# nv-tlabs/DefTet

Measured on AMD Instinct MI355X. Metric: M tet-point tests/s (fwd+bwd) at res=70, 100k queries, higher is better.
Workload: dtype f32

## Files before the change

### deftet_amd/csrc/point_in_tet.hip

```cpp
#pragma clang fp contract(off)

#include <stdlib.h>

#include <algorithm>
#include <type_traits>
#include <vector>

#include "common.hpp"

namespace deftet {
namespace pit {

constexpr float kBig = 1048576.0f;
constexpr float kTau = 1.0f / 128.0f;
constexpr float kMargin = 1.0f / 64.0f;
constexpr float kWMin = 9.3132257e-10f;
constexpr int kMiss = 0x7F7F7F7F;
constexpr int kMaxG = 112;
constexpr int kMaxBins = 15 * 1024;
constexpr int kHitOverflow = -2;

constexpr int kHitPad = 64;
__host__ __device__ inline int hit_pad(int B) { return (B + kHitPad - 1) / kHitPad * kHitPad; }
__host__ __device__ inline size_t hit_cnt_off(int B, int T) { return (size_t)B * T * 2; }
// ... 662 lines not shown
    PHASE_MARK(12);
    SPAN_MARK(1);
    if (keep) return;
    __syncthreads();
    for (int i = tid; i < n; i += kSortThreads) {
        const float4 q = src[source_of(i)];
        dst[atomicAdd(&cnt[(cell_of(q.y, oy, iy, G) - cyLo) * GxP + cell_of(q.x, ox, ix, Gx)], 1)] = q;
    }
}

__device__ __forceinline__ void irregular_queries_tail(const Planes &P, int t, int b, int Q, const float *__restrict__ pts,
                                                       const int *__restrict__ counters, const int *__restrict__ irregQ, int *result)
{
    const int n = counters[b * 4 + 1];
    for (int k = 0; k < n; ++k) {
        const int q = irregQ[(size_t)b * Q + k];
        const float *p = pts + ((size_t)b * Q + q) * 3;
        if (accept(P, p[0], p[1], p[2])) atomicMin(&result[(size_t)b * Q + q], t);
    }
}

#ifndef PIT_WAVES
#define PIT_WAVES 5
#endif


struct TetBox {
    float lo[3], hi[3], w;
};
__device__ __forceinline__ bool classify(const float *v, const Planes &P, TetBox &bx)
{
#pragma unroll
    for (int k = 0; k < 3; ++k) {
        bx.lo[k] = fminf(fminf(v[k], v[3 + k]), fminf(v[6 + k], v[9 + k]));
        bx.hi[k] = fmaxf(fmaxf(v[k], v[3 + k]), fmaxf(v[6 + k], v[9 + k]));
    }
    bx.w = fmaxf(fmaxf(bx.hi[0] - bx.lo[0], bx.hi[1] - bx.lo[1]), bx.hi[2] - bx.lo[2]);
    const float big = fmaxf(fmaxf(fmaxf(fabsf(bx.lo[0]), fabsf(bx.hi[0])), fmaxf(fabsf(bx.lo[1]), fabsf(bx.hi[1]))),
                            fmaxf(fabsf(bx.lo[2]), fabsf(bx.hi[2])));
    const float thr = kTau * ((bx.w * bx.w) * bx.w);
    const bool cond = fabsf(P.dv[0]) >= thr && fabsf(P.dv[1]) >= thr && fabsf(P.dv[2]) >= thr && fabsf(P.dv[3]) >= thr;
    return big <= kBig && (P.sv == 0u || P.sv == 15u) && bx.w >= kWMin && cond;
}

struct CellBox {
    int cx0, cx1, cy0, cy1, cz0, cz1;
};

__device__ __forceinline__ float4 ld_f4_hint(const float4 *p, bool nt)
{
    if (!nt) return *p;
    typedef float f4v __attribute__((ext_vector_type(4)));
    const f4v x = __builtin_nontemporal_load(reinterpret_cast<const f4v *>(p));
    return make_float4(x[0], x[1], x[2], x[3]);
}
struct DenseTets {
    typedef const float *__restrict__ Arg;
    typedef const float *Ref;
    typedef const float *__restrict__ RefArg;
    const float *tet;
    __host__ __device__ __forceinline__ DenseTets(const float *p) : tet(p) {}
    __device__ __forceinline__ Ref at(int b, int T, int t) const { return tet + ((size_t)b * T + t) * 12; }
    __device__ __forceinline__ Ref at_flat(long long i, int ) const { return tet + i * 12; }
    template <bool NT = false>
    __device__ __forceinline__ static void get3(Ref r, float4 &a, float4 &bq, float4 &c)
    {
        const float4 *src = reinterpret_cast<const float4 *>(r);
        a = ld_f4_hint(src, NT); bq = ld_f4_hint(src + 1, NT); c = ld_f4_hint(src + 2, NT);
    }
    template <bool NT = false>
    __device__ __forceinline__ static void get4(Ref r, float (&v)[12])
    {
        float4 a, bq, c;
        get3<NT>(r, a, bq, c);
        v[0] = a.x; v[1] = a.y; v[2] = a.z; v[3] = a.w;
        v[4] = bq.x; v[5] = bq.y; v[6] = bq.z; v[7] = bq.w;
        v[8] = c.x; v[9] = c.y; v[10] = c.z; v[11] = c.w;
    }
    __device__ __forceinline__ static void get(Ref r, float (&v)[12])
    {
#pragma unroll
        for (int k = 0; k < 12; ++k) v[k] = r[k];
    }
};
struct IndexedTets {
    const float *pos;
    const int *idx;
    long long idxStride;
    int V;
    typedef IndexedTets Arg;
    struct Ref {
        const float *p;
        const int *ix;
        unsigned V;
    };
    typedef Ref RefArg;
    __device__ __forceinline__ Ref at(int b, int T, int t) const
    {
        (void)T;
        return Ref{pos + (size_t)b * (size_t)V * 3, idx + (size_t)b * idxStride + (size_t)t * 4, (unsigned)V};
    }
    __device__ __forceinline__ Ref at_flat(long long i, int T) const { return at((int)(i / T), T, (int)(i % T)); }
    template <bool NT = false>
    __device__ __forceinline__ static void get4(const Ref &r, float (&v)[12])
    {
        const int4 c = *reinterpret_cast<const int4 *>(r.ix);
        const int ci[4] = {c.x, c.y, c.z, c.w};
#pragma unroll
        for (int k = 0; k < 4; ++k) {
            const unsigned u = (unsigned)ci[k];
            if (u < r.V) {
                const float *p = r.p + (size_t)u * 3;
                v[3 * k] = p[0]; v[3 * k + 1] = p[1]; v[3 * k + 2] = p[2];
            } else {
                v[3 * k] = v[3 * k + 1] = v[3 * k + 2] = __int_as_float(0x7FC00000);
            }
        }
    }
    template <bool NT = false>
    __device__ __forceinline__ static void get3(const Ref &r, float4 &a, float4 &bq, float4 &c)
    {
        float v[12];
        get4(r, v);
        a = make_float4(v[0], v[1], v[2], v[3]); bq = make_float4(v[4], v[5], v[6], v[7]); c = make_float4(v[8], v[9], v[10], v[11]);
    }
    __device__ __forceinline__ static void get(const Ref &r, float (&v)[12]) { get4(r, v); }
};
__global__ __launch_bounds__(256) void k_idx_check(const int4 *__restrict__ idx, long long n, unsigned V, int *bad)
{
    const long long i = (long long)blockIdx.x * blockDim.x + threadIdx.x;
    if (i >= n) return;
    const int4 c = idx[i];
    if ((unsigned)c.x >= V || (unsigned)c.y >= V || (unsigned)c.z >= V || (unsigned)c.w >= V) *bad = 1;
}

template <class TS_, bool F>
struct TetCfg {
    typedef TS_ TS;
    static constexpr bool flag = F;
};

template <class TS>
__global__ __launch_bounds__(256, PIT_WAVES) void k_tet_scan(typename TS::Arg tet, int T, int Q,
                                                  const float *__restrict__ gparam, int G, int Gx, const int *__restrict__ table,
                                                  long long cellStride, const float4 *__restrict__ sortedQ, int *result, int *counters,
                                                  int *irregT, int2 *hits, const float *__restrict__ pts,
                                                  const int *__restrict__ irregQ, int *ucount, int hpad, int4 *spill)
{
    if (ucount && blockIdx.x == 0 && __builtin_amdgcn_readfirstlane(threadIdx.x) == 0) {
        ucount[blockIdx.y] = 0;
        ucount[hpad + blockIdx.y] = 0;
        ucount[2 * hpad + blockIdx.y] = 0;
    }
    const int b = blockIdx.y;
    const int nblk = gridDim.x;
    const int per = (nblk + 7) >> 3;
    const int vb = (blockIdx.x & 7) * per + (blockIdx.x >> 3);
    const int t = vb * blockDim.x + threadIdx.x;
    if (vb >= nblk || t >= T) return;
    const TS ts(tet);
    float v[12];
    if constexpr (std::is_same<TS, DenseTets>::value) {
        const float4 *src = reinterpret_cast<const float4 *>(tet + ((size_t)b * T + t) * 12);
        float4 a = src[0], bq = src[1], c = src[2];
        v[0] = a.x; v[1] = a.y; v[2] = a.z; v[3] = a.w;
        v[4] = bq.x; v[5] = bq.y; v[6] = bq.z; v[7] = bq.w;
        v[8] = c.x; v[9] = c.y; v[10] = c.z; v[11] = c.w;
    } else {
        TS::get4(ts.at(b, T, t), v);
    }
    Planes P;
    make_planes(v, P);
    TetBox bx;
    const bool regular = classify(v, P, bx);
    int hq[kRecSlots + kSpillSlots] = {-1, -1, -1, -1, -1, -1};
    int hcnt = 0;
    if (!regular) {
        int k = atomicAdd(&counters[b * 4 + 0], 1);
        irregT[(size_t)b * T + k] = t;
        if (hits) hits[(size_t)b * T + t] = make_int2(-1, kHitOverflow);
        irregular_queries_tail(P, t, b, Q, pts, counters, irregQ, result);
        return;
    }
    const Grid g = load_grid(gparam + b * kGridWords);
    const float m = bx.w * kMargin;
    float elo[3], ehi[3];
#pragma unroll
    for (int k = 0; k < 3; ++k) {
        elo[k] = bx.lo[k] - m;
        ehi[k] = bx.hi[k] + m;
    }
    if (ehi[0] < g.lo[0] || elo[0] > g.hi[0] || ehi[1] < g.lo[1] || elo[1] > g.hi[1] || ehi[2] < g.lo[2] || elo[2] > g.hi[2]) {
        if (hits) hits[(size_t)b * T + t] = make_int2(-1, -1);
        irregular_queries_tail(P, t, b, Q, pts, counters, irregQ, result);
        return;
    }
    const int cx0 = cell_of(elo[0], g.o[0], g.inv[0], Gx), cx1 = cell_of(ehi[0], g.o[0], g.inv[0], Gx);
    const int cy0 = cell_of(elo[1], g.o[1], g.inv[1], G), cy1 = cell_of(ehi[1], g.o[1], g.inv[1], G);
    const int cz0 = cell_of(elo[2], g.o[2], g.inv[2], G), cz1 = cell_of(ehi[2], g.o[2], g.inv[2], G);
    if (wide_tet(cx0, cx1, cy0, cy1, cz0, cz1, g)) {
        int k = atomicAdd(&counters[b * 4 + 0], 1);
        irregT[(size_t)b * T + k] = t;
        if (hits) hits[(size_t)b * T + t] = make_int2(-1, kHitOverflow);
        irregular_queries_tail(P, t, b, Q, pts, counters, irregQ, result);
        return;
    }
    const int Gp = table_pitch(G);
    const int *tb = table + (size_t)b * cellStride;
    const float4 *sq = sortedQ + (size_t)b * Q;
    int *res = result + (size_t)b * Q;
    for (int cz = cz0; cz <= cz1; ++cz)
        for (int cy = cy0; cy <= cy1; ++cy) {
            const int s = tb[table_off(cz, cx0, cy, Gx, Gp)], e = tb[table_off(cz, cx1 + 1, cy, Gx, Gp)];
            for (int j = s; j < e; ++j) {
                const float4 q = sq[j];
                if (q.x >= elo[0] && q.x <= ehi[0] && q.y >= elo[1] && q.y <= ehi[1] && q.z >= elo[2] && q.z <= ehi[2] &&
                    accept(P, q.x, q.y, q.z)) {
                    const int qi = __float_as_int(q.w);
                    atomicMin(&res[qi], t);
#pragma unroll
                    for (int k = 0; k < kRecSlots + kSpillSlots; ++k)
                        if (hcnt == k) hq[k] = qi;
                    ++hcnt;
                }
            }
        }
    if (hits) put_hit_record(hits, spill, (size_t)b * T + t, hq, hcnt, counters, gridDim.y, b, t);
    irregular_queries_tail(P, t, b, Q, pts, counters, irregQ, result);
}

struct Filter {
    float N[4][3];
    float C[4];
    float twoEmax;
};

typedef unsigned long long lanemask_t;
__device__ __forceinline__ int sel(lanemask_t m, int if_set, int if_clear)
{
    int d;
    asm("v_cndmask_b32_e64 %0, %1, %2, %3" : "=v"(d) : "v"(if_clear), "v"(if_set), "s"(m));
    return d;
}
__device__ __forceinline__ unsigned sel(lanemask_t m, unsigned if_set, unsigned if_clear)
{
    return (unsigned)sel(m, (int)if_set, (int)if_clear);
}
__device__ __forceinline__ lanemask_t mask_of(bool c) { return __builtin_amdgcn_ballot_w64(c); }


template <typename T>
__device__ __forceinline__ T ld_off(const void *base, unsigned byte_off)
{
    return *reinterpret_cast<const T *>(static_cast<const char *>(base) + byte_off);
}
struct __attribute__((packed, aligned(4))) int4u { int x, y, z, w; };
__device__ __forceinline__ int4u ld_off_u4(const void *base, unsigned byte_off)
{
    return *reinterpret_cast<const int4u *>(static_cast<const char *>(base) + byte_off);
}

__device__ __forceinline__ void atomic_smin_off(int *base, unsigned byte_off, int v)
{
    asm volatile("s_nop 4\n\tglobal_atomic_smin %0, %1, %2" ::"v"(byte_off), "v"(v), "s"(base) : "memory");
}
template <typename T>
__device__ __forceinline__ T *uniform_ptr(T *p)
{
    const unsigned long long v = reinterpret_cast<unsigned long long>(p);
    const unsigned lo = __builtin_amdgcn_readfirstlane((unsigned)v), hi = __builtin_amdgcn_readfirstlane((unsigned)(v >> 32));
    return reinterpret_cast<T *>(((unsigned long long)hi << 32) | lo);
}
typedef int i32x4 __attribute__((ext_vector_type(4)));
typedef int i32x2s __attribute__((ext_vector_type(2)));
typedef float f32x4 __attribute__((ext_vector_type(4)));
__device__ __forceinline__ void stream_store(float4 *p, const float4 v)
{
    const f32x4 x = {v.x, v.y, v.z, v.w};
    __builtin_nontemporal_store(x, reinterpret_cast<f32x4 *>(p));
}
__device__ __forceinline__ void stream_store(float *p, float v) { __builtin_nontemporal_store(v, p); }
#ifndef PIT_SCAN_TET_NT
#define PIT_SCAN_TET_NT 0
#endif
#ifndef PIT_BWD_TET_NT
#define PIT_BWD_TET_NT 0
#endif
#ifndef PIT_BWD_REV
#define PIT_BWD_REV 0
#endif
#ifndef PIT_REC_NT
#define PIT_REC_NT 1
#endif
__device__ __forceinline__ void store_rec(int2 *p, const int2 v)
{
    if (PIT_REC_NT) {
        const i32x2s x = {v.x, v.y};
        __builtin_nontemporal_store(x, reinterpret_cast<i32x2s *>(p));
    } else {
        *p = v;
    }
}
__device__ __forceinline__ int2 stream_load(const int2 *p)
{
    const i32x2s x = __builtin_nontemporal_load(reinterpret_cast<const i32x2s *>(p));
    return make_int2(x.x, x.y);
}
__device__ __forceinline__ void store_b128_off(void *base, unsigned byte_off, int x, int y, int z, int w)
{
    const i32x4 v = {x, y, z, w};
    asm volatile("s_nop 4\n\tglobal_store_dwordx4 %0, %1, %2\n\ts_nop 2" ::"v"(byte_off), "v"(v), "s"(base) : "memory");
}

typedef int i32x2 __attribute__((ext_vector_type(2)));
__device__ __forceinline__ void store_b64_off(void *base, unsigned byte_off, int x, int y)
{
    const i32x2 v = {x, y};
    asm volatile("s_nop 4\n\tglobal_store_dwordx2 %0, %1, %2\n\ts_nop 2" ::"v"(byte_off), "v"(v), "s"(base) : "memory");
}

template <class TS>
__device__ __noinline__ void exact_rescan(typename TS::RefArg tv, int t, const int *__restrict__ tb, const float4 *__restrict__ sq,
                                          int *res, int G, int Gx, int cx0, int cx1, int cy0, int cy1, int cz0, int cz1,
                                          float m, int *counters, int nB, int b, int2 *hits, int4 *spill, size_t idx)
{
    float vv[12];
    TS::get(tv, vv);
    Planes P;
    make_planes(vv, P);
    float elo[3], ehi[3];
#pragma unroll
    for (int k = 0; k < 3; ++k) {
        elo[k] = fminf(fminf(vv[k], vv[3 + k]), fminf(vv[6 + k], vv[9 + k])) - m;
        ehi[k] = fmaxf(fmaxf(vv[k], vv[3 + k]), fmaxf(vv[6 + k], vv[9 + k])) + m;
    }
    const int Gp = table_pitch(G);
    int hq[kRecSlots + kSpillSlots] = {-1, -1, -1, -1, -1, -1};
    int hcnt = 0;
    for (int cz = cz0; cz <= cz1; ++cz)
// ... 1287 lines not shown
        if (threadIdx.x == 0) {
            const float tot = (wsum[0] + wsum[1]) + (wsum[2] + wsum[3]);
            if (tot != 0.f) unsafeAtomicAdd(&missSum[b], tot);
        }
    }
}

template <class TS>
__global__ __launch_bounds__(256) void k_bary_bwd_gather(typename TS::Arg tet, const float *__restrict__ pts,
                                                         const float *__restrict__ grad_w, const int *__restrict__ head,
                                                         const int *__restrict__ next, int T, int Q, float *grad_tet,
                                                         float *grad_pts, int accumulate, const float *__restrict__ gocc,
                                                         const float *__restrict__ missSum, float *grad_pred)
{
    const int b = blockIdx.y;
    const int t = blockIdx.x * blockDim.x + threadIdx.x;
    if (t >= T) return;
    float acc[12];
#pragma unroll
    for (int k = 0; k < 12; ++k) acc[k] = 0.f;
    int q = head[(size_t)b * T + t];
    float gp = (grad_pred && t == 0) ? missSum[b] : 0.f;
    if (q >= 0) {
        float4 t0, t1, t2;
        TS::get3(TS(tet).at(b, T, t), t0, t1, t2);
        const float A[3] = {t0.x, t0.y, t0.z}, Bv[3] = {t0.w, t1.x, t1.y}, Cv[3] = {t1.z, t1.w, t2.x}, D[3] = {t2.y, t2.z, t2.w};
        float vab[3], vac[3], vad[3], vbc[3], vbd[3];
#pragma unroll
        for (int k = 0; k < 3; ++k) {
            vab[k] = Bv[k] - A[k]; vac[k] = Cv[k] - A[k]; vad[k] = D[k] - A[k];
            vbc[k] = Cv[k] - Bv[k]; vbd[k] = D[k] - Bv[k];
        }
        float na[3], nb[3], nc[3], nd[3];
        cross3(vbd, vbc, na);
        cross3(vac, vad, nb);
        cross3(vad, vab, nc);
        cross3(vab, vac, nd);
        const float v6 = 1.0f / (vab[0] * nb[0] + vab[1] * nb[1] + vab[2] * nb[2]);
        while (q >= 0) {
            const size_t i = (size_t)b * Q + q;
            const float *pp = pts + i * 3;
            const float4 g = reinterpret_cast<const float4 *>(grad_w)[i];
            const int qn = next[i];
            float vap[3], vbp[3];
#pragma unroll
            for (int k = 0; k < 3; ++k) { vap[k] = pp[k] - A[k]; vbp[k] = pp[k] - Bv[k]; }
            float w[4];
            w[0] = (vbp[0] * na[0] + vbp[1] * na[1] + vbp[2] * na[2]) * v6;
            w[1] = (vap[0] * nb[0] + vap[1] * nb[1] + vap[2] * nb[2]) * v6;
            w[2] = (vap[0] * nc[0] + vap[1] * nc[1] + vap[2] * nc[2]) * v6;
            w[3] = (vap[0] * nd[0] + vap[1] * nd[1] + vap[2] * nd[2]) * v6;
            float G3[3];
#pragma unroll
            for (int k = 0; k < 3; ++k) G3[k] = (g.x * na[k] + g.y * nb[k] + g.z * nc[k] + g.w * nd[k]) * v6;
#pragma unroll
            for (int vtx = 0; vtx < 4; ++vtx)
#pragma unroll
                for (int k = 0; k < 3; ++k) acc[vtx * 3 + k] += -w[vtx] * G3[k];
            if (grad_pts) { grad_pts[i * 3] = G3[0]; grad_pts[i * 3 + 1] = G3[1]; grad_pts[i * 3 + 2] = G3[2]; }
            if (grad_pred) gp += gocc[i];
            q = qn;
        }
    }
    if (grad_pred) grad_pred[(size_t)b * T + t] = accumulate ? grad_pred[(size_t)b * T + t] + gp : gp;
    float4 *dst = reinterpret_cast<float4 *>(grad_tet + ((size_t)b * T + t) * 12);
    float4 o0 = make_float4(acc[0], acc[1], acc[2], acc[3]), o1 = make_float4(acc[4], acc[5], acc[6], acc[7]),
           o2 = make_float4(acc[8], acc[9], acc[10], acc[11]);
    if (accumulate) {
        float4 p0 = dst[0], p1 = dst[1], p2 = dst[2];
        o0.x += p0.x; o0.y += p0.y; o0.z += p0.z; o0.w += p0.w;
        o1.x += p1.x; o1.y += p1.y; o1.z += p1.z; o1.w += p1.w;
        o2.x += p2.x; o2.y += p2.y; o2.z += p2.z; o2.w += p2.w;
    }
    dst[0] = o0; dst[1] = o1; dst[2] = o2;
}

constexpr int kMissParts = 64;

struct TetGrad {
    float A[3], Bv[3];
    float na[3], nb[3], nc[3], nd[3];
    float v6;
};
template <class TS>
__device__ __forceinline__ void tet_grad_setup(typename TS::Ref r, TetGrad &g)
{
    float4 t0, t1, t2;
    TS::template get3<PIT_BWD_TET_NT != 0>(r, t0, t1, t2);
    const float C[3] = {t1.z, t1.w, t2.x}, D[3] = {t2.y, t2.z, t2.w};
    g.A[0] = t0.x; g.A[1] = t0.y; g.A[2] = t0.z; g.Bv[0] = t0.w; g.Bv[1] = t1.x; g.Bv[2] = t1.y;
    float vab[3], vac[3], vad[3], vbc[3], vbd[3];
#pragma unroll
    for (int k = 0; k < 3; ++k) {
        vab[k] = g.Bv[k] - g.A[k]; vac[k] = C[k] - g.A[k]; vad[k] = D[k] - g.A[k];
        vbc[k] = C[k] - g.Bv[k]; vbd[k] = D[k] - g.Bv[k];
    }
    cross3(vbd, vbc, g.na);
    cross3(vac, vad, g.nb);
    cross3(vad, vab, g.nc);
    cross3(vab, vac, g.nd);
    g.v6 = 1.0f / (vab[0] * g.nb[0] + vab[1] * g.nb[1] + vab[2] * g.nb[2]);
}
__device__ __forceinline__ void tet_grad_add(const TetGrad &g, const float *pp, const float4 gw, float *acc, float *G3)
{
    float vap[3], vbp[3];
#pragma unroll
    for (int k = 0; k < 3; ++k) { vap[k] = pp[k] - g.A[k]; vbp[k] = pp[k] - g.Bv[k]; }
    float w[4];
    w[0] = (vbp[0] * g.na[0] + vbp[1] * g.na[1] + vbp[2] * g.na[2]) * g.v6;
    w[1] = (vap[0] * g.nb[0] + vap[1] * g.nb[1] + vap[2] * g.nb[2]) * g.v6;
    w[2] = (vap[0] * g.nc[0] + vap[1] * g.nc[1] + vap[2] * g.nc[2]) * g.v6;
    w[3] = (vap[0] * g.nd[0] + vap[1] * g.nd[1] + vap[2] * g.nd[2]) * g.v6;
#pragma unroll
    for (int k = 0; k < 3; ++k) G3[k] = (gw.x * g.na[k] + gw.y * g.nb[k] + gw.z * g.nc[k] + gw.w * g.nd[k]) * g.v6;
#pragma unroll
    for (int vtx = 0; vtx < 4; ++vtx)
#pragma unroll
        for (int k = 0; k < 3; ++k) acc[vtx * 3 + k] += -w[vtx] * G3[k];
}

__device__ __forceinline__ float mem_read_f32(float *p) { return __int_as_float(atomicOr(reinterpret_cast<int *>(p), 0)); }
__device__ __forceinline__ void mem_write_f32(float *p, float v)
{
    const int old = atomicExch(reinterpret_cast<int *>(p), __float_as_int(v));
    asm volatile("" ::"v"(old));
}

constexpr int kMissStride = 80;

constexpr long long kRescanOrderedSteps = 16384;
template <class TS>
__device__ __forceinline__ bool bwd_rescan(typename TS::Arg tet, const float *__restrict__ pts, const float *__restrict__ cond,
                                        const float *__restrict__ grad_w, const float *__restrict__ gocc, float *grad_pts,
                                        bool want_pred, const int *__restrict__ ulist, int b, int T, int Q, int nU,
                                        unsigned long long need, int t, float (*park)[256])
{
    const int tid = threadIdx.x, lane = tid & 63;
    const int *__restrict__ lst = ulist + (size_t)b * Q;
    bool parked = false;
    while (need) {
        const int L = __ffsll((long long)need) - 1;
        need &= need - 1;
        const int tL = __shfl(t, L);
        const float tLf = (float)tL;
        int m = 0;
        auto next_hit = [&](int cur, bool count) {
            int best = 0x7FFFFFFF;
            for (int base = 0; base < nU; base += 64) {
                const int e = base + lane;
                const int q = e < nU ? lst[e] : -1;
                const bool mine = q > cur && cond[(size_t)b * Q + q] == tLf;
                if (mine) best = min(best, q);
                if (count) m += __popcll(__ballot(mine));
            }
#pragma unroll
            for (int off = 32; off > 0; off >>= 1) best = min(best, __shfl_xor(best, off));
            return best;
        };
        int best = next_hit(-1, true);
        if (m == 0) continue;
        const bool ordered = (long long)m * ((nU + 63) >> 6) <= kRescanOrderedSteps;
        float part[13];
#pragma unroll
        for (int k = 0; k < 13; ++k) part[k] = 0.f;
        TetGrad g;
        tet_grad_setup<TS>(TS(tet).at(b, T, tL), g);
        for (int base = 0;;) {
            int q;
            bool mine;
            if (ordered) {
                if (best == 0x7FFFFFFF) break;
                q = best;
                mine = true;
            } else {
                if (base >= nU) break;
                const int e = base + lane;
                q = e < nU ? lst[e] : -1;
                mine = q >= 0 && cond[(size_t)b * Q + q] == tLf;
                base += 64;
            }
            if (mine) {
                const size_t i = (size_t)b * Q + q;
                float G3[3];
                tet_grad_add(g, pts + i * 3, reinterpret_cast<const float4 *>(grad_w)[i], part, G3);
                if (grad_pts) { grad_pts[i * 3] = G3[0]; grad_pts[i * 3 + 1] = G3[1]; grad_pts[i * 3 + 2] = G3[2]; }
                if (want_pred) part[12] += gocc[i];
            }
            if (ordered) best = next_hit(best, false);
        }
        if (!ordered) {
#pragma unroll
            for (int k = 0; k < 13; ++k) {
                float v = part[k];
#pragma unroll
                for (int off = 32; off > 0; off >>= 1) v += __shfl_xor(v, off);
                part[k] = v;
            }
        }
        if (lane == L) {
#pragma unroll
            for (int k = 0; k < 13; ++k) park[k][tid] = part[k];
            parked = true;
        }
    }
    return parked;
}

#ifndef PIT_BWD_WAVES
#define PIT_BWD_WAVES 7
#endif
template <class C>
__global__ __launch_bounds__(256, PIT_BWD_WAVES) void k_bary_bwd_hits(typename C::TS::Arg tet, const float *__restrict__ pts,
                                                       const float *__restrict__ cond, const float *__restrict__ grad_w,
                                                       const int2 *__restrict__ hits, int T, int Q, float *grad_tet,
                                                       float *grad_pts, int accumulate, const float *__restrict__ gocc,
                                                       float *grad_pred, float *missPart, int nMissParts, int *hitWords,
                                                       const int *__restrict__ ulist, int pad, const int4 *__restrict__ spill, int pin,
                                                       unsigned long long *rowMask)
{
    __shared__ float wsum[4];
    __shared__ float s_vals[kMissStride];
    __shared__ int s_last;
    __shared__ __attribute__((aligned(16))) float s_buf[13 * 256];
    float4(*s_rows)[192] = reinterpret_cast<float4(*)[192]>(s_buf);
    float(*s_park)[256] = reinterpret_cast<float(*)[256]>(s_buf);
    typedef typename C::TS TS;
    constexpr bool SPARSE = C::flag;
    const int2 sb = shape_block(pin);
    const int b = sb.x, bx = PIT_BWD_REV ? (int)gridDim.x - 1 - sb.y : sb.y, tid = threadIdx.x, lane = tid & 63;
    const bool side = grad_pred && bx < nMissParts;
    float missPartial = 0.f;
    if (side) {
        float gm = 0.f;
        for (int q = bx * blockDim.x + tid; q < Q; q += nMissParts * blockDim.x)
            if (cond[(size_t)b * Q + q] < 0.f) gm += gocc[(size_t)b * Q + q];
#pragma unroll
        for (int off = 32; off > 0; off >>= 1) gm += __shfl_xor(gm, off);
        if (lane == 0) wsum[tid >> 6] = gm;
        __syncthreads();
        missPartial = __int_as_float(__builtin_amdgcn_readfirstlane(__float_as_int((wsum[0] + wsum[1]) + (wsum[2] + wsum[3]))));
    }
    const int t = bx * blockDim.x + tid;
    const bool live = t < T;
    int2 h = live ? stream_load(hits + (size_t)b * T + t) : make_int2(-1, -1);
    const bool spilled = h.y != kHitOverflow && h.x >= 0 && (h.x & kHitSpilled) != 0;
    if (spilled) h.x &= ~kHitSpilled;
    bool parked = false;
    const int nU = hitWords[b];
    if (nU > 0) {
        const bool anyQ = hitWords[2 * pad + b] != 0;
        const unsigned long long need = __ballot(live && (h.y == kHitOverflow || anyQ));
        if (need) parked = bwd_rescan<TS>(tet, pts, cond, grad_w, gocc, grad_pts, grad_pred != nullptr, ulist, b, T, Q, nU, need, t, s_park);
    }
    float acc[12];
#pragma unroll
    for (int k = 0; k < 12; ++k) acc[k] = 0.f;
    float gp = 0.f;
    if (h.x >= 0 && h.y != kHitOverflow) {
        TetGrad g;
        tet_grad_setup<TS>(TS(tet).at(b, T, t), g);
        unsigned hu[8] = {(unsigned)h.x, (unsigned)h.y, ~0u, ~0u, ~0u, ~0u, ~0u, ~0u};
        const float tf = (float)t;
        auto add_hit = [&](int q) {
            if (q < 0) return;
            const size_t i = (size_t)b * Q + q;
            const float c = cond[i], go = grad_pred ? gocc[i] : 0.f;
            const float pq[3] = {pts[i * 3], pts[i * 3 + 1], pts[i * 3 + 2]};
            const float4 gw = reinterpret_cast<const float4 *>(grad_w)[i];
            const bool won = c == tf;
            float G3[3], a2[12];
#pragma unroll
            for (int k = 0; k < 12; ++k) a2[k] = acc[k];
            tet_grad_add(g, pq, gw, a2, G3);
#pragma unroll
            for (int k = 0; k < 12; ++k) acc[k] = won ? a2[k] : acc[k];
            if (won && grad_pts) { grad_pts[i * 3] = G3[0]; grad_pts[i * 3 + 1] = G3[1]; grad_pts[i * 3 + 2] = G3[2]; }
            gp = won ? gp + go : gp;
        };
#define DEFTET_CSWAP(a, b) { const unsigned lo_ = min(hu[a], hu[b]), hi_ = max(hu[a], hu[b]); hu[a] = lo_; hu[b] = hi_; }
        if (!__any(spilled)) {
            DEFTET_CSWAP(0, 1)
#pragma unroll 1
            for (int k = 0; k < 2 && __any(hu[0] != ~0u); ++k) {
                add_hit((int)hu[0]);
                hu[0] = hu[1]; hu[1] = ~0u;
            }
        } else {
            if (spilled) {
                const int4 h2 = spill[(size_t)b * T + t];
                hu[2] = (unsigned)h2.x; hu[3] = (unsigned)h2.y; hu[4] = (unsigned)h2.z; hu[5] = (unsigned)h2.w;
            }
            DEFTET_CSWAP(0, 1) DEFTET_CSWAP(2, 3) DEFTET_CSWAP(4, 5) DEFTET_CSWAP(6, 7)
            DEFTET_CSWAP(0, 2) DEFTET_CSWAP(1, 3) DEFTET_CSWAP(4, 6) DEFTET_CSWAP(5, 7)
            DEFTET_CSWAP(1, 2) DEFTET_CSWAP(5, 6) DEFTET_CSWAP(0, 4) DEFTET_CSWAP(3, 7)
            DEFTET_CSWAP(1, 5) DEFTET_CSWAP(2, 6)
            DEFTET_CSWAP(1, 4) DEFTET_CSWAP(3, 6)
            DEFTET_CSWAP(2, 4) DEFTET_CSWAP(3, 5)
            DEFTET_CSWAP(3, 4)
#pragma unroll 1
            for (int k = 0; k < 6 && __any(hu[0] != ~0u); ++k) {
                add_hit((int)hu[0]);
#pragma unroll
                for (int j = 0; j < 7; ++j) hu[j] = hu[j + 1];
                hu[7] = ~0u;
            }
        }
#undef DEFTET_CSWAP
    }
    if (parked) {
#pragma unroll
        for (int k = 0; k < 12; ++k) acc[k] += s_park[k][tid];
        gp += s_park[12][tid];
    }
    if (nU > 0) __syncthreads();
    if (live) {
        const bool deferred = grad_pred && t == 0;
        if (grad_pred && !deferred) stream_store(grad_pred + (size_t)b * T + t, accumulate ? grad_pred[(size_t)b * T + t] + gp : gp);
    }
    {
        const int w = tid >> 6;
        const int t0 = t - lane;
        const bool has = live && ((h.x >= 0 && h.y != kHitOverflow) || parked);
        const unsigned long long hm = SPARSE ? __ballot(has) : 0ull;
        const int slot = SPARSE ? __popcll(hm & ((1ull << lane) - 1ull)) : lane;
        if (!SPARSE || has) {
            s_rows[w][slot * 3] = make_float4(acc[0], acc[1], acc[2], acc[3]);
            s_rows[w][slot * 3 + 1] = make_float4(acc[4], acc[5], acc[6], acc[7]);
            s_rows[w][slot * 3 + 2] = make_float4(acc[8], acc[9], acc[10], acc[11]);
        }
        if (SPARSE && lane == 0 && t0 < T) rowMask[(size_t)b * ((T + 63) >> 6) + (t0 >> 6)] = hm;
        __syncthreads();
        float4 *dst = reinterpret_cast<float4 *>(grad_tet + ((size_t)b * T + t0) * 12);
        const int nRow = (SPARSE ? __popcll(hm) : min(64, T - t0)) * 3;
#pragma unroll
        for (int k = 0; k < 3; ++k) {
            const int j = k * 64 + lane;
            if (j < nRow) {
                float4 o = s_rows[w][j];
                if (accumulate && !SPARSE) { const float4 p = dst[j]; o.x += p.x; o.y += p.y; o.z += p.z; o.w += p.w; }
                stream_store(dst + j, o);
            }
        }
    }
    if (!side) return;
    float *mp = missPart + (size_t)b * kMissStride;
    int *ticket = hitWords + pad + b;
    if (tid == 0) {
        mem_write_f32(mp + bx, missPartial);
        if (bx == 0) mem_write_f32(mp + kMissParts, gp);
        __builtin_amdgcn_s_waitcnt(0);
        s_last = atomicAdd(ticket, 1) == nMissParts - 1;
    }
    __syncthreads();
    if (!s_last) return;
    if (tid <= kMissParts) s_vals[tid] = (tid < nMissParts || tid == kMissParts) ? mem_read_f32(mp + tid) : 0.f;
    __syncthreads();
    if (tid == 0) {
        float tot = 0.f;
        for (int k = 0; k < kMissParts; ++k) tot += s_vals[k];
        tot += s_vals[kMissParts];
        float *dst = grad_pred + (size_t)b * T;
        *dst = accumulate ? *dst + tot : tot;
        atomicExch(ticket, 0);
    }
}

__global__ __launch_bounds__(256) void k_paste_fwd(const float *__restrict__ pred, float *cond, float *out, int T, int Q,
                                                   int clamp_inplace)
{
    const int b = blockIdx.y;
    const int q = blockIdx.x * blockDim.x + threadIdx.x;
    if (q >= Q) return;
    const size_t i = (size_t)b * Q + q;
    float c = cond[i];
    if (c < 0) {
        c = 0.f;
        if (clamp_inplace) cond[i] = 0.f;
    }
    out[i] = pred[(size_t)b * T + (long long)c];
}

__global__ __launch_bounds__(256) void k_paste_bwd(const float *__restrict__ cond, const float *__restrict__ gout,
                                                   float *gpred, int T, int Q)
{
    const int b = blockIdx.y;
    const int q = blockIdx.x * blockDim.x + threadIdx.x;
    const bool live = q < Q;
// ... 348 lines not shown
{
    int n = 0;
    DEFTET_HIP(hipOccupancyMaxActiveBlocksPerMultiprocessor(&n, (const void *)deftet::pit::k_tet_scan_wave<deftet::pit::TetCfg<deftet::pit::DenseTets, false>>, 256, 0)); out8[0] = n;
    DEFTET_HIP(hipOccupancyMaxActiveBlocksPerMultiprocessor(&n, (const void *)deftet::pit::k_tet_scan_pair<deftet::pit::TetCfg<deftet::pit::DenseTets, false>>, 256, 0)); out8[1] = n;
    DEFTET_HIP(hipOccupancyMaxActiveBlocksPerMultiprocessor(&n, (const void *)deftet::pit::k_tet_scan_slab<deftet::pit::TetCfg<deftet::pit::DenseTets, false>>, 256, 0)); out8[2] = n;
    hipFuncAttributes a;
    DEFTET_HIP(hipFuncGetAttributes(&a, (const void *)deftet::pit::k_tet_scan_wave<deftet::pit::TetCfg<deftet::pit::DenseTets, false>>));
    out8[3] = (int)a.sharedSizeBytes; out8[4] = a.numRegs; out8[5] = (int)a.maxDynamicSharedSizeBytes;
    hipDeviceProp_t pr;
    DEFTET_HIP(hipGetDeviceProperties(&pr, 0));
    out8[6] = (int)pr.sharedMemPerMultiprocessor; out8[7] = (int)pr.sharedMemPerBlock;
    return DEFTET_OK;
}
extern "C" int deftet_debug_span_read(unsigned long long *out, int n_waves)
{
    DEFTET_CHECK_ARG(out && n_waves > 0 && n_waves <= deftet::pit::kPhaseWaves, "bad argument");
    DEFTET_HIP(hipMemcpyFromSymbol(out, HIP_SYMBOL(deftet::pit::g_span), (size_t)n_waves * 16));
    return DEFTET_OK;
}
extern "C" int deftet_debug_reason_read(unsigned long long *out8, int reset)
{
    DEFTET_HIP(hipMemcpyFromSymbol(out8, HIP_SYMBOL(deftet::pit::g_reason), 64));
    if (reset) {
        unsigned long long z[8] = {0};
        DEFTET_HIP(hipMemcpyToSymbol(HIP_SYMBOL(deftet::pit::g_reason), z, 64));
    }
    return DEFTET_OK;
}
extern "C" int deftet_debug_phase_read(unsigned long long *out16, int reset)
{
    std::vector<unsigned long long> h((size_t)kPhaseWaves * 16);
    DEFTET_HIP(hipMemcpyFromSymbol(h.data(), HIP_SYMBOL(deftet::pit::g_phase), h.size() * sizeof(unsigned long long)));
    for (int i = 0; i < 16; ++i) out16[i] = 0;
    for (size_t w = 0; w < (size_t)kPhaseWaves; ++w)
        for (int i = 0; i < 16; ++i) out16[i] += h[w * 16 + i];
    if (reset) {
        std::fill(h.begin(), h.end(), 0ull);
        DEFTET_HIP(hipMemcpyToSymbol(HIP_SYMBOL(deftet::pit::g_phase), h.data(), h.size() * sizeof(unsigned long long)));
    }
    return DEFTET_OK;
}
#endif

constexpr long long kDenseQueriesPerTet = 2;
extern "C" size_t deftet_point_in_tet_bwd_workspace_bytes(int B, int T, int Q)
{
    if (B <= 0 || T < 0 || Q < 0) return 0;
    const size_t lists = align_up((size_t)B * T * 4, 256) + align_up((size_t)B * Q * 4, 256) + align_up((size_t)B * 4, 256);
    const size_t miss = align_up((size_t)B * kMissStride * 4, 256);
    return lists > miss ? lists : miss;
}

static bool tets_null(const float *tet) { return tet == nullptr; }
static bool tets_null(const IndexedTets &s) { return s.pos == nullptr || s.idx == nullptr; }
static bool tets_misaligned(const float *tet) { return ((uintptr_t)tet & 15) != 0; }
static bool tets_misaligned(const IndexedTets &s) { return ((uintptr_t)s.idx & 15) != 0 || ((uintptr_t)s.pos & 3) != 0; }

template <class TS>
static int pit_bwd(typename TS::Arg tet, const float *pts, const float *cond, const float *grad_w, float *grad_tet, float *grad_pts,
                   const float *grad_occ, float *grad_pred, const int32_t *hit_buf, int B, int T, int Q, int accumulate, void *workspace,
                   size_t workspace_bytes, void *stream_)
{
    DEFTET_CHECK_ARG(B >= 0 && T >= 0 && Q >= 0, "negative size");
    DEFTET_CHECK_ARG(B <= 65535, "n_batch=%d exceeds 65535", B);
    DEFTET_CHECK_ARG((grad_occ == nullptr) == (grad_pred == nullptr), "grad_occ and grad_pred must be given together");
    hipStream_t st = as_stream(stream_);
    if (B == 0) return DEFTET_OK;
    if (grad_pts && Q > 0) DEFTET_HIP(hipMemsetAsync(grad_pts, 0, (size_t)B * Q * 12, st));
    if (T == 0) return DEFTET_OK;
    DEFTET_CHECK_ARG(grad_tet && ((uintptr_t)grad_tet & 15) == 0, "grad_tet null or not 16-byte aligned");
    if (Q == 0) {
        if (!accumulate) {
            DEFTET_HIP(hipMemsetAsync(grad_tet, 0, (size_t)B * T * 48, st));
            if (grad_pred) DEFTET_HIP(hipMemsetAsync(grad_pred, 0, (size_t)B * T * 4, st));
        }
        return DEFTET_OK;
    }
    DEFTET_CHECK_ARG(!tets_null(tet) && pts && cond && grad_w, "null pointer");
    DEFTET_CHECK_ARG(!tets_misaligned(tet) && ((uintptr_t)grad_w & 15) == 0, "tet/grad_w must be 16-byte aligned");
    const bool dense = (long long)Q > kDenseQueriesPerTet * (long long)T && workspace && ((uintptr_t)workspace & 255) == 0 &&
                       workspace_bytes >= deftet_point_in_tet_bwd_workspace_bytes(B, T, Q);
    if (hit_buf && !dense) {
        DEFTET_CHECK_ARG(((uintptr_t)hit_buf & 15) == 0, "hit_buf must be 16-byte aligned");
        float *missPart = nullptr;
        if (grad_pred) {
            DEFTET_CHECK_ARG(workspace && workspace_bytes >= (size_t)B * kMissStride * 4, "workspace needed for the miss sums (80 floats per shape)");
            missPart = static_cast<float *>(workspace);
        }
        const int tblocks = (T + 255) / 256, nMissParts = tblocks < kMissParts ? tblocks : kMissParts;
        int32_t *words = const_cast<int32_t *>(hit_buf) + hit_cnt_off(B, T);
        typedef TetCfg<TS, false> Dense;
        DEFTET_LAUNCH(k_bary_bwd_hits<Dense>, dim3(tblocks, B), dim3(256), st, tet, pts, cond, grad_w, (const int2 *)hit_buf, T, Q,
                      grad_tet, grad_pts, accumulate, grad_occ, grad_pred, missPart, nMissParts, words,
                      (const int *)(hit_buf + hit_list_off(B, T)), hit_pad(B), (const int4 *)(hit_buf + hit_spill_off(B, T, Q)), pin_shapes(Q),
                      (unsigned long long *)nullptr);
    } else if (workspace) {
        const size_t need = deftet_point_in_tet_bwd_workspace_bytes(B, T, Q);
        DEFTET_CHECK_ARG(workspace_bytes >= need && ((uintptr_t)workspace & 255) == 0,
                         "backward workspace too small (%zu < %zu) or misaligned", workspace_bytes, need);
        char *w = static_cast<char *>(workspace);
        int *head = reinterpret_cast<int *>(w);
        int *next = reinterpret_cast<int *>(w + align_up((size_t)B * T * 4, 256));
        float *missSum = reinterpret_cast<float *>(w + align_up((size_t)B * T * 4, 256) + align_up((size_t)B * Q * 4, 256));
        DEFTET_HIP(hipMemsetAsync(head, 0xFF, (size_t)B * T * 4, st));
        if (grad_pred) DEFTET_HIP(hipMemsetAsync(missSum, 0, (size_t)B * 4, st));
        DEFTET_LAUNCH(k_hit_link, dim3((Q + 256 * kLinkPer - 1) / (256 * kLinkPer), B), dim3(256), st, cond, T, Q, head, next,
                      grad_occ, missSum);
        DEFTET_LAUNCH(k_bary_bwd_gather<TS>, dim3((T + 255) / 256, B), dim3(256), st, tet, pts, grad_w, head, next, T, Q,
                      grad_tet, grad_pts, accumulate, grad_occ, missSum, grad_pred);
    } else {
        if (!accumulate) DEFTET_HIP(hipMemsetAsync(grad_tet, 0, (size_t)B * T * 48, st));
        DEFTET_LAUNCH(k_bary_bwd<TS>, dim3((Q + 255) / 256, B), dim3(256), st, tet, pts, cond, grad_w, T, Q, grad_tet,
                      grad_pts);
        if (grad_pred) {
            if (!accumulate) DEFTET_HIP(hipMemsetAsync(grad_pred, 0, (size_t)B * T * 4, st));
            DEFTET_LAUNCH(k_paste_bwd, dim3((Q + 255) / 256, B), dim3(256), st, cond, grad_occ, grad_pred, T, Q);
        }
    }
    return DEFTET_OK;
}
extern "C" int deftet_point_in_tet_bwd_f32(const float *tet, const float *pts, const float *cond, const float *grad_w,
                                           float *grad_tet, float *grad_pts, const float *grad_occ, float *grad_pred,
                                           const int32_t *hit_buf, int B, int T, int Q, int accumulate, void *workspace,
                                           size_t workspace_bytes, void *stream_)
{
    return pit_bwd<DenseTets>(tet, pts, cond, grad_w, grad_tet, grad_pts, grad_occ, grad_pred, hit_buf, B, T, Q, accumulate, workspace,
                              workspace_bytes, stream_);
}

extern "C" size_t deftet_point_in_tet_bwd_to_vertices_workspace_bytes(int B, int T, int Q)
{
    if (B <= 0 || T < 0 || Q < 0) return 0;
    return align_up((size_t)B * T * 48, 256) + align_up((size_t)B * ((T + 63) / 64) * 8, 256) +
           align_up(deftet_point_in_tet_bwd_workspace_bytes(B, T, Q), 256);
}

template <class TS>
static int pit_bwd_to_vertices(typename TS::Arg tet, const float *pts, const float *cond, const float *grad_w, const float *grad_occ,
                               const int32_t *hit_buf, const int32_t *csr_offsets, const int32_t *csr_slots, int idx_batch,
                               float *grad_pos, float *grad_pts, float *grad_pred, int B, int V, int T, int Q, int accumulate,
                               void *workspace, size_t workspace_bytes, void *stream_)
{
    DEFTET_CHECK_ARG(B >= 0 && V >= 0 && T >= 0 && Q >= 0, "negative size");
    DEFTET_CHECK_ARG(B <= 65535, "n_batch=%d exceeds 65535", B);
    DEFTET_CHECK_ARG((grad_occ == nullptr) == (grad_pred == nullptr), "grad_occ and grad_pred must be given together");
    DEFTET_CHECK_ARG(idx_batch == 1 || idx_batch == B, "CSR batch must be 1 or n_batch (got %d)", idx_batch);
    hipStream_t st = as_stream(stream_);
    if (B == 0) return DEFTET_OK;
    DEFTET_CHECK_ARG(V == 0 || grad_pos, "null grad_pos");
    if (T == 0 || Q == 0 || V == 0) {
        if (grad_pts && Q > 0) DEFTET_HIP(hipMemsetAsync(grad_pts, 0, (size_t)B * Q * 12, st));
        if (!accumulate) {
            if (V > 0) DEFTET_HIP(hipMemsetAsync(grad_pos, 0, (size_t)B * V * 12, st));
            if (grad_pred && T > 0) DEFTET_HIP(hipMemsetAsync(grad_pred, 0, (size_t)B * T * 4, st));
        }
        return DEFTET_OK;
    }
    DEFTET_CHECK_ARG(!tets_null(tet) && pts && cond && grad_w && csr_offsets && csr_slots, "null pointer");
    DEFTET_CHECK_ARG(!tets_misaligned(tet) && ((uintptr_t)grad_w & 15) == 0, "tet/grad_w must be 16-byte aligned");
    const size_t need = deftet_point_in_tet_bwd_to_vertices_workspace_bytes(B, T, Q);
    DEFTET_CHECK_ARG(workspace && workspace_bytes >= need && ((uintptr_t)workspace & 255) == 0,
                     "workspace null, misaligned or too small (%zu < %zu)", workspace_bytes, need);
    Arena A(workspace, workspace_bytes);
    float *rows = A.take<float>((size_t)B * T * 12);
    unsigned long long *rowMask = A.take<unsigned long long>((size_t)B * ((T + 63) / 64));
    const size_t innerBytes = deftet_point_in_tet_bwd_workspace_bytes(B, T, Q);
    void *inner = A.take<char>(innerBytes);
    const bool dense = (long long)Q > kDenseQueriesPerTet * (long long)T;
    if (hit_buf && !dense) {
        DEFTET_CHECK_ARG(((uintptr_t)hit_buf & 15) == 0, "hit_buf must be 16-byte aligned");
        if (grad_pts) DEFTET_HIP(hipMemsetAsync(grad_pts, 0, (size_t)B * Q * 12, st));
        const int tblocks = (T + 255) / 256, nMissParts = tblocks < kMissParts ? tblocks : kMissParts;
        int32_t *words = const_cast<int32_t *>(hit_buf) + hit_cnt_off(B, T);
        typedef TetCfg<TS, true> Sparse;
        DEFTET_LAUNCH(k_bary_bwd_hits<Sparse>, dim3(tblocks, B), dim3(256), st, tet, pts, cond, grad_w, (const int2 *)hit_buf, T, Q,
                      rows, grad_pts, accumulate, grad_occ, grad_pred, static_cast<float *>(inner), nMissParts, words,
                      (const int *)(hit_buf + hit_list_off(B, T)), hit_pad(B), (const int4 *)(hit_buf + hit_spill_off(B, T, Q)), pin_shapes(Q),
                      rowMask);
        return vtx::gather_bwd_rows(rows, rowMask, csr_offsets, csr_slots, grad_pos, B, V, T, idx_batch, accumulate, st);
    }
    if (accumulate) DEFTET_HIP(hipMemsetAsync(rows, 0, (size_t)B * T * 48, st));
    const int rc = pit_bwd<TS>(tet, pts, cond, grad_w, rows, grad_pts, grad_occ, grad_pred, hit_buf, B, T, Q, accumulate, inner,
                               innerBytes, stream_);
    if (rc != DEFTET_OK) return rc;
    return vtx::gather_bwd_rows(rows, nullptr, csr_offsets, csr_slots, grad_pos, B, V, T, idx_batch, accumulate, st);
}
extern "C" int deftet_point_in_tet_bwd_to_vertices_f32(const float *tet, const float *pts, const float *cond, const float *grad_w,
                                                       const float *grad_occ, const int32_t *hit_buf, const int32_t *csr_offsets,
                                                       const int32_t *csr_slots, int idx_batch, float *grad_pos, float *grad_pts,
                                                       float *grad_pred, int B, int V, int T, int Q, int accumulate, void *workspace,
                                                       size_t workspace_bytes, void *stream_)
{
    return pit_bwd_to_vertices<DenseTets>(tet, pts, cond, grad_w, grad_occ, hit_buf, csr_offsets, csr_slots, idx_batch, grad_pos, grad_pts,
                                          grad_pred, B, V, T, Q, accumulate, workspace, workspace_bytes, stream_);
}

static int pit_check_indexed(const float *pos, const int32_t *tet_idx, int idx_batch, int B, int V, int T)
{
    DEFTET_CHECK_ARG(B >= 0 && V >= 0 && T >= 0, "negative size (B=%d V=%d T=%d)", B, V, T);
    DEFTET_CHECK_ARG(idx_batch == 1 || idx_batch == B, "idx_batch must be 1 or n_batch (got %d, n_batch %d)", idx_batch, B);
    DEFTET_CHECK_ARG(((uintptr_t)tet_idx & 15) == 0, "tet_idx must be 16-byte aligned");
    DEFTET_CHECK_ARG(((uintptr_t)pos & 3) == 0, "pos must be 4-byte aligned");
    if ((long long)V * 3 >= (1ll << 31)) return set_error(DEFTET_ELIMIT, "n_vertex=%d: vertex offsets exceed 2^31", V);
    if (B > 0 && T > 0) DEFTET_CHECK_ARG(tet_idx && (pos || V == 0), "null pos/tet_idx pointer");
    return DEFTET_OK;
}
static IndexedTets make_indexed(const float *pos, const int32_t *tet_idx, int idx_batch, int V, int T)
{
    IndexedTets s;
    s.pos = pos;
    s.idx = tet_idx;
    s.idxStride = idx_batch == 1 ? 0 : (long long)T * 4;
    s.V = V;
    return s;
}
static int flag_bad_indices(const int32_t *tet_idx, int idx_batch, int V, int T, int32_t *bad_flag, hipStream_t st)
{
    const long long n = (long long)idx_batch * T;
    if (!bad_flag || n == 0) return DEFTET_OK;
    DEFTET_LAUNCH(k_idx_check, dim3((unsigned)((n + 255) / 256)), dim3(256), st, reinterpret_cast<const int4 *>(tet_idx), n, (unsigned)V, bad_flag);
    return DEFTET_OK;
}

extern "C" int deftet_point_in_tet_indexed_f32(const float *pos, const int32_t *tet_idx, int idx_batch, const float *pts, float *cond,
                                               float *bary, const float *pred, float *occ, int32_t *hit_buf, int B, int V, int T, int Q,
                                               int algo, const int32_t *tet_order, const float *query_box_in, float *query_box_out,
                                               int32_t *query_box_misses, int32_t *bad_flag, void *workspace, size_t workspace_bytes,
                                               void *stream_)
{
    int rc = pit_check_indexed(pos, tet_idx, idx_batch, B, V, T);
    if (rc != DEFTET_OK) return rc;
    DEFTET_CHECK_ARG(!query_box_in || query_box_in != query_box_out, "query_box_in and query_box_out must not alias");
    rc = pit_check(reinterpret_cast<const float *>(tet_idx), pts, cond, bary, pred, occ, hit_buf, B, T, Q, algo, workspace);
    if (rc != DEFTET_OK || B == 0) return rc;
    rc = flag_bad_indices(tet_idx, idx_batch, V, T, bad_flag, as_stream(stream_));
    if (rc != DEFTET_OK || Q == 0) return rc;
    return pit_forward_checked<IndexedTets>(make_indexed(pos, tet_idx, idx_batch, V, T), pts, cond, bary, pred, occ, hit_buf, B, T,
                                            Q, algo, workspace, workspace_bytes, stream_, tet_order, query_box_in, query_box_out,
                                            query_box_misses);
}

extern "C" int deftet_point_in_tet_indexed_scan_f32(const float *pos, const int32_t *tet_idx, int idx_batch, const float *pts, float *cond,
                                                    float *bary, const float *pred, float *occ, int32_t *hit_buf, int B, int V, int T,
                                                    int Q, int algo, const int32_t *tet_order, int32_t *bad_flag, void *workspace,
                                                    size_t workspace_bytes, void *stream_)
{
    int rc = pit_check_indexed(pos, tet_idx, idx_batch, B, V, T);
    if (rc != DEFTET_OK) return rc;
    DEFTET_CHECK_ARG(algo != DEFTET_PIT_BRUTE, "scan needs a binned algo");
    rc = pit_check(reinterpret_cast<const float *>(tet_idx), pts, cond, bary, pred, occ, hit_buf, B, T, Q, algo, workspace);
    if (rc != DEFTET_OK || B == 0) return rc;
    rc = flag_bad_indices(tet_idx, idx_batch, V, T, bad_flag, as_stream(stream_));
    if (rc != DEFTET_OK || Q == 0) return rc;
// ... 46 lines not shown
```

Measured before the change: 1.077 billion.

## Prefetch hit query data and split tet load to overlap latency in backward

In the backward hits kernel, the tet vertex load is split into a begin/finish pair, so the index or corner fetch is issued early and the gradient setup happens later. Both hit records' query data (cond, grad_occ, points, grad_w) are fetched up front behind a scheduling barrier. The common two-hit path is unrolled without the ballot loop, and the spilled path now handles hits in pairs. The aim is to hide global-memory latency by issuing the independent loads together, at the cost of more live registers. 32-bit byte offsets are used for the loads, so a Q < 2^27 guard is added.

```diff
diff --git a/deftet_amd/csrc/point_in_tet.hip b/deftet_amd/csrc/point_in_tet.hip
--- a/deftet_amd/csrc/point_in_tet.hip
+++ b/deftet_amd/csrc/point_in_tet.hip
@@ -768,6 +768,15 @@
 #pragma unroll
         for (int k = 0; k < 12; ++k) v[k] = r[k];
     }
+    struct Pre { float4 a, bq, c; };
+    template <bool NT = false>
+    __device__ __forceinline__ static Pre begin(Ref r)
+    {
+        Pre p;
+        get3<NT>(r, p.a, p.bq, p.c);
+        return p;
+    }
+    __device__ __forceinline__ static void finish(Ref, const Pre &p, float4 &a, float4 &bq, float4 &c) { a = p.a; bq = p.bq; c = p.c; }
 };
 struct IndexedTets {
     const float *pos;
@@ -790,7 +799,19 @@
     template <bool NT = false>
     __device__ __forceinline__ static void get4(const Ref &r, float (&v)[12])
     {
-        const int4 c = *reinterpret_cast<const int4 *>(r.ix);
+        get_corners(r, *reinterpret_cast<const int4 *>(r.ix), v);
+    }
+    typedef int4 Pre;
+    template <bool NT = false>
+    __device__ __forceinline__ static Pre begin(const Ref &r) { return *reinterpret_cast<const int4 *>(r.ix); }
+    __device__ __forceinline__ static void finish(const Ref &r, const Pre &p, float4 &a, float4 &bq, float4 &c)
+    {
+        float v[12];
+        get_corners(r, p, v);
+        a = make_float4(v[0], v[1], v[2], v[3]); bq = make_float4(v[4], v[5], v[6], v[7]); c = make_float4(v[8], v[9], v[10], v[11]);
+    }
+    __device__ __forceinline__ static void get_corners(const Ref &r, const int4 c, float (&v)[12])
+    {
         const int ci[4] = {c.x, c.y, c.z, c.w};
 #pragma unroll
         for (int k = 0; k < 4; ++k) {
@@ -941,6 +962,7 @@
     return *reinterpret_cast<const T *>(static_cast<const char *>(base) + byte_off);
 }
 struct __attribute__((packed, aligned(4))) int4u { int x, y, z, w; };
+struct __attribute__((packed, aligned(4))) float3u { float x, y, z; };
 __device__ __forceinline__ int4u ld_off_u4(const void *base, unsigned byte_off)
 {
     return *reinterpret_cast<const int4u *>(static_cast<const char *>(base) + byte_off);
@@ -2394,11 +2416,8 @@
     float na[3], nb[3], nc[3], nd[3];
     float v6;
 };
-template <class TS>
-__device__ __forceinline__ void tet_grad_setup(typename TS::Ref r, TetGrad &g)
-{
-    float4 t0, t1, t2;
-    TS::template get3<PIT_BWD_TET_NT != 0>(r, t0, t1, t2);
+__device__ __forceinline__ void tet_grad_make(const float4 t0, const float4 t1, const float4 t2, TetGrad &g)
+{
     const float C[3] = {t1.z, t1.w, t2.x}, D[3] = {t2.y, t2.z, t2.w};
     g.A[0] = t0.x; g.A[1] = t0.y; g.A[2] = t0.z; g.Bv[0] = t0.w; g.Bv[1] = t1.x; g.Bv[2] = t1.y;
     float vab[3], vac[3], vad[3], vbc[3], vbd[3];
@@ -2412,6 +2431,13 @@
     cross3(vad, vab, g.nc);
     cross3(vab, vac, g.nd);
     g.v6 = 1.0f / (vab[0] * g.nb[0] + vab[1] * g.nb[1] + vab[2] * g.nb[2]);
+}
+template <class TS>
+__device__ __forceinline__ void tet_grad_setup(typename TS::Ref r, TetGrad &g)
+{
+    float4 t0, t1, t2;
+    TS::template get3<PIT_BWD_TET_NT != 0>(r, t0, t1, t2);
+    tet_grad_make(t0, t1, t2, g);
 }
 __device__ __forceinline__ void tet_grad_add(const TetGrad &g, const float *pp, const float4 gw, float *acc, float *G3)
 {
@@ -2569,39 +2595,64 @@
     for (int k = 0; k < 12; ++k) acc[k] = 0.f;
     float gp = 0.f;
     if (h.x >= 0 && h.y != kHitOverflow) {
-        TetGrad g;
-        tet_grad_setup<TS>(TS(tet).at(b, T, t), g);
+        const typename TS::Ref ref = TS(tet).at(b, T, t);
+        const typename TS::Pre pre = TS::template begin<PIT_BWD_TET_NT != 0>(ref);
         unsigned hu[8] = {(unsigned)h.x, (unsigned)h.y, ~0u, ~0u, ~0u, ~0u, ~0u, ~0u};
         const float tf = (float)t;
-        auto add_hit = [&](int q) {
-            if (q < 0) return;
-            const size_t i = (size_t)b * Q + q;
-            const float c = cond[i], go = grad_pred ? gocc[i] : 0.f;
-            const float pq[3] = {pts[i * 3], pts[i * 3 + 1], pts[i * 3 + 2]};
-            const float4 gw = reinterpret_cast<const float4 *>(grad_w)[i];
-            const bool won = c == tf;
+        struct HitIn {
+            float c, go, pq[3];
+            float4 gw;
+        };
+        const float *condB = cond + (size_t)b * Q, *goB = (grad_pred ? gocc : cond) + (size_t)b * Q;
+        const float *ptsB = pts + (size_t)b * Q * 3, *gwB = grad_w + (size_t)b * Q * 4;
+        auto fetch = [&](unsigned qu, HitIn &x) {
+            if ((int)qu < 0) qu = 0;
+            x.c = ld_off<float>(condB, qu * 4u);
+            x.go = ld_off<float>(goB, qu * 4u);
+            const float3u p = ld_off<float3u>(ptsB, qu * 12u);
+            x.pq[0] = p.x; x.pq[1] = p.y; x.pq[2] = p.z;
+            x.gw = ld_off<float4>(gwB, qu * 16u);
+        };
+        auto pin = [](const HitIn &x) {
+            asm volatile("" ::"v"(x.c), "v"(x.go), "v"(x.pq[0]), "v"(x.pq[1]), "v"(x.pq[2]), "v"(x.gw.x), "v"(x.gw.y), "v"(x.gw.z), "v"(x.gw.w));
+        };
+        TetGrad g;
+        auto add_hit = [&](unsigned qu, const HitIn &x) {
+            if ((int)qu < 0) return;
+            const size_t i = (size_t)b * Q + qu;
+            const bool won = x.c == tf;
             float G3[3], a2[12];
 #pragma unroll
             for (int k = 0; k < 12; ++k) a2[k] = acc[k];
-            tet_grad_add(g, pq, gw, a2, G3);
+            tet_grad_add(g, x.pq, x.gw, a2, G3);
 #pragma unroll
             for (int k = 0; k < 12; ++k) acc[k] = won ? a2[k] : acc[k];
             if (won && grad_pts) { grad_pts[i * 3] = G3[0]; grad_pts[i * 3 + 1] = G3[1]; grad_pts[i * 3 + 2] = G3[2]; }
-            gp = won ? gp + go : gp;
+            gp = won ? gp + x.go : gp;
+        };
+        auto make_g = [&]() {
+            float4 t0, t1, t2;
+            TS::finish(ref, pre, t0, t1, t2);
+            tet_grad_make(t0, t1, t2, g);
         };
 #define DEFTET_CSWAP(a, b) { const unsigned lo_ = min(hu[a], hu[b]), hi_ = max(hu[a], hu[b]); hu[a] = lo_; hu[b] = hi_; }
         if (!__any(spilled)) {
             DEFTET_CSWAP(0, 1)
-#pragma unroll 1
-            for (int k = 0; k < 2 && __any(hu[0] != ~0u); ++k) {
-                add_hit((int)hu[0]);
-                hu[0] = hu[1]; hu[1] = ~0u;
-            }
+            HitIn x0, x1;
+            fetch(hu[0], x0);
+            fetch(hu[1], x1);
+            __builtin_amdgcn_sched_barrier(0);
+            make_g();
+            pin(x0);
+            pin(x1);
+            add_hit(hu[0], x0);
+            add_hit(hu[1], x1);
         } else {
             if (spilled) {
                 const int4 h2 = spill[(size_t)b * T + t];
                 hu[2] = (unsigned)h2.x; hu[3] = (unsigned)h2.y; hu[4] = (unsigned)h2.z; hu[5] = (unsigned)h2.w;
             }
+            make_g();
             DEFTET_CSWAP(0, 1) DEFTET_CSWAP(2, 3) DEFTET_CSWAP(4, 5) DEFTET_CSWAP(6, 7)
             DEFTET_CSWAP(0, 2) DEFTET_CSWAP(1, 3) DEFTET_CSWAP(4, 6) DEFTET_CSWAP(5, 7)
             DEFTET_CSWAP(1, 2) DEFTET_CSWAP(5, 6) DEFTET_CSWAP(0, 4) DEFTET_CSWAP(3, 7)
@@ -2610,11 +2661,17 @@
             DEFTET_CSWAP(2, 4) DEFTET_CSWAP(3, 5)
             DEFTET_CSWAP(3, 4)
 #pragma unroll 1
-            for (int k = 0; k < 6 && __any(hu[0] != ~0u); ++k) {
-                add_hit((int)hu[0]);
-#pragma unroll
-                for (int j = 0; j < 7; ++j) hu[j] = hu[j + 1];
-                hu[7] = ~0u;
+            for (int k = 0; k < 3 && __any(hu[0] != ~0u); ++k) {
+                HitIn x0, x1;
+                fetch(hu[0], x0);
+                fetch(hu[1], x1);
+                pin(x0);
+                pin(x1);
+                add_hit(hu[0], x0);
+                add_hit(hu[1], x1);
+#pragma unroll
+                for (int j = 0; j < 6; ++j) hu[j] = hu[j + 2];
+                hu[6] = hu[7] = ~0u;
             }
         }
 #undef DEFTET_CSWAP
@@ -3129,6 +3186,7 @@
                        workspace_bytes >= deftet_point_in_tet_bwd_workspace_bytes(B, T, Q);
     if (hit_buf && !dense) {
         DEFTET_CHECK_ARG(((uintptr_t)hit_buf & 15) == 0, "hit_buf must be 16-byte aligned");
+        DEFTET_CHECK_ARG(Q < (1 << 27), "n_query=%d exceeds 2^27 (no forward writes records for it)", Q);
         float *missPart = nullptr;
         if (grad_pred) {
             DEFTET_CHECK_ARG(workspace && workspace_bytes >= (size_t)B * kMissStride * 4, "workspace needed for the miss sums (80 floats per shape)");
@@ -3216,6 +3274,7 @@
     const bool dense = (long long)Q > kDenseQueriesPerTet * (long long)T;
     if (hit_buf && !dense) {
         DEFTET_CHECK_ARG(((uintptr_t)hit_buf & 15) == 0, "hit_buf must be 16-byte aligned");
+        DEFTET_CHECK_ARG(Q < (1 << 27), "n_query=%d exceeds 2^27 (no forward writes records for it)", Q);
         if (grad_pts) DEFTET_HIP(hipMemsetAsync(grad_pts, 0, (size_t)B * Q * 12, st));
         const int tblocks = (T + 255) / 256, nMissParts = tblocks < kMissParts ? tblocks : kMissParts;
         int32_t *words = const_cast<int32_t *>(hit_buf) + hit_cnt_off(B, T);
```

Measured after the change: 1.078 billion (median of 3 runs). No clear change (+0.0%).
